# cornell-zhang/HiSparse

Measured on AMD Instinct MI355X. Metric: SpMV GBPS (8 B per non-zero per SpMV, sw/benchmark.cpp:312-346), higher is better.
Workload: dtype u32 (Q8.24 fixed point, u64 row sums)

## Files before the change

hisparse_amd/csrc/spmv_bitmap.hip:

```cpp
#include <hip/hip_runtime.h>

#include <cstdio>
#include <cstdlib>
#include <vector>

#include "spmv_device.h"
#include "spmv_kernels.h"

namespace hisparse {
namespace dev {

namespace {

constexpr int kBmThreads = kWaveLanes * kBitmapWaves;
constexpr int kBatch = 8;
constexpr uint32_t kInvalidOffset = 0x80000000u;
constexpr uint32_t kRsrcFlags = 0x00020000u;
constexpr int kXCopyPasses = (kBitmapMaxXLdsGroups * (kBitmapGroupCols / 4) + kBmThreads - 1) / kBmThreads;

typedef const __attribute__((address_space(4))) WaveSeg* WaveSegTable;

template <bool kFloat>
struct Batch {
    uint32_t v[kBatch], xv[kBatch];
    uint64_t m[kBatch];
};

typedef const __attribute__((address_space(3))) uint32_t* LdsWords;

template <typename T>
__device__ __forceinline__ T* uniform_ptr(T* p) {
    const uint64_t v = reinterpret_cast<uint64_t>(p);
    const uint32_t hi = static_cast<uint32_t>(__builtin_amdgcn_readfirstlane(static_cast<uint32_t>(v >> 32)));
    const uint32_t lo = static_cast<uint32_t>(__builtin_amdgcn_readfirstlane(static_cast<uint32_t>(v)));
    return reinterpret_cast<T*>((static_cast<uint64_t>(hi) << 32) | lo);
}

template <bool kFloat, int kAblate, bool kXLds>
__device__ __forceinline__ typename Rows<kFloat>::sum_t bitmap_row_run(const uint64_t* mp, const uint32_t*& vp, const uint32_t* x, uint32_t num_cols,
                                                                       uint32_t col0, uint32_t steps, uint32_t lane, bool have_first,
                                                                       const uint32_t (&first_masks)[4], LdsWords xs_run, uint64_t* stamps = nullptr) {
    using R = Rows<kFloat>;
    typename R::sum_t acc = 0;
    const auto vr = __builtin_amdgcn_make_buffer_rsrc(uniform_ptr(const_cast<uint32_t*>(vp)), 0, 0x7fffffffu, kRsrcFlags);
    uint32_t xk[kBatch];
#pragma unroll
    for (int k = 0; k < kBatch; ++k) xk[k] = (lane + k * kBitmapGroupCols) * 4u;
    uint32_t voff = 0;
    const auto mr = __builtin_amdgcn_make_buffer_rsrc(uniform_ptr(const_cast<uint64_t*>(mp)), 0, steps * 8u, kRsrcFlags);
    uint32_t moff = lane < 2 * kBatch ? lane * 4u : kInvalidOffset;
    constexpr uint32_t kBatchMaskBytes = kBatch * 8u;
    uint32_t mcur = have_first ? first_masks[0] : __builtin_amdgcn_raw_buffer_load_b32(mr, moff, 0, 0);
    uint32_t m1 = have_first ? first_masks[1] : __builtin_amdgcn_raw_buffer_load_b32(mr, moff + kBatchMaskBytes, 0, 0);
    uint32_t m2 = have_first ? first_masks[2] : __builtin_amdgcn_raw_buffer_load_b32(mr, moff + 2 * kBatchMaskBytes, 0, 0);
    uint32_t m3 = have_first ? first_masks[3] : __builtin_amdgcn_raw_buffer_load_b32(mr, moff + 3 * kBatchMaskBytes, 0, 0);
    auto issue = [&](Batch<kFloat>& b, uint32_t bb) {
        constexpr uint32_t sel = 0;
        const uint32_t xc = min(col0 + bb * (kBatch * kBitmapGroupCols), num_cols);
        const auto xr = __builtin_amdgcn_make_buffer_rsrc(const_cast<uint32_t*>(x + xc), 0, (num_cols - xc) * 4u, kRsrcFlags);
#pragma unroll
        for (int k = 0; k < kBatch; ++k) {
            const uint32_t lo = __builtin_amdgcn_readlane(mcur, sel + 2 * k), hi = __builtin_amdgcn_readlane(mcur, sel + 2 * k + 1);
            b.m[k] = (static_cast<uint64_t>(hi) << 32) | lo;
            const uint32_t off = __builtin_amdgcn_mbcnt_hi(hi, __builtin_amdgcn_mbcnt_lo(lo, 0)) * 4u;
            b.v[k] = (kAblate & 1) ? off : __builtin_amdgcn_raw_buffer_load_b32(vr, off, voff, (kAblate & 256) ? 2 : 0);
            if constexpr (kXLds) b.xv[k] = (kAblate & 2) ? lo : xs_run[(bb * kBatch + k) * kBitmapGroupCols + lane];
            else b.xv[k] = (kAblate & 2) ? lo : __builtin_amdgcn_raw_buffer_load_b32(xr, xk[k], 0, 0);
            const uint32_t set = static_cast<uint32_t>(__builtin_popcountll(b.m[k]));
            asm("s_lshl2_add_u32 %0, %1, %2" : "=s"(voff) : "s"(set), "s"(__builtin_amdgcn_readfirstlane(voff)) : "scc");
// ... 49 lines not shown
        rotate_masks(bb + 2);
        issue(A, bb + 2);
        consume(B);
        rotate_masks(bb + 3);
        issue(B, bb + 3);
    }
    vp += voff / 4u;
    return acc;
}

template <bool kFloat, int kAblate, bool kXLds = false>
__global__ __launch_bounds__(kBmThreads) void spmv_bitmap_kernel(const uint8_t* __restrict__ image, const Block* __restrict__ blocks,
                                                                const Unit* __restrict__ units, const uint32_t* __restrict__ x, uint32_t num_cols,
                                                                uint32_t* __restrict__ out, int32_t row_part_filter,
                                                                const uint32_t* __restrict__ part_heads, uint64_t* __restrict__ timeline,
                                                                uint32_t x_lds_offset, CarriedCombine carry) {
    using R = Rows<kFloat>;
    using acc_t = typename R::acc_t;
    extern __shared__ __attribute__((aligned(16))) uint8_t lds[];
    acc_t* ys = reinterpret_cast<acc_t*>(lds);
    const uint32_t tid = threadIdx.x;
    const uint32_t lane = tid & (kWaveLanes - 1);
    const uint32_t wave = __builtin_amdgcn_readfirstlane(tid / kWaveLanes);
    uint64_t* stamps = (kAblate & 64) ? timeline + (static_cast<size_t>(blockIdx.x) * kBitmapWaves + wave) * 8 : nullptr;
    auto stamp = [&](int i, uint32_t dep) {
        if (!(kAblate & 64)) return;
        uint64_t t;
        asm volatile("s_memrealtime %0\n\ts_waitcnt lgkmcnt(0)" : "=s"(t) : "s"(dep));
        if (lane == 0) stamps[i] = t;
    };
    stamp(0, wave);
    uint32_t wg = blockIdx.x;
    if ((gridDim.x & 7u) == 0) wg = (blockIdx.x & 7u) * (gridDim.x >> 3) + (blockIdx.x >> 3);
    if (carry.partial) carried_combine<kFloat, kBmThreads>(carry, blockIdx.x, gridDim.x, tid);
    uint32_t bi = wg;
    if (row_part_filter >= 0) {
        bi = ((const __attribute__((address_space(4))) uint32_t*)part_heads)[static_cast<uint32_t>(row_part_filter) * gridDim.x + wg];
        if (bi == kNoBlock) return;
    }
    bool first_block = true;
    uint32_t staged_col0 = 0, staged_groups = 0;
    for (uint32_t next = 0;; bi = next) {
        const BlockTable blk = (BlockTable)(blocks + bi);
        next = (row_part_filter >= 0 && blk->next_part > static_cast<uint32_t>(row_part_filter)) ? 0u : blk->next;
        const uint32_t nrows = blk->nrows, out0 = blk->out_offset;
        const uint32_t* hdr = reinterpret_cast<const uint32_t*>(units) + (static_cast<size_t>(bi) * kBitmapWaves + wave) * (kBitmapRunSlots * 16);
        const uint32_t seg_word = hdr[min(lane, 15u)];
        uint32_t first_masks[4];
#pragma unroll
        for (int b = 0; b < 4; ++b) first_masks[b] = hdr[16 + 16 * b + (lane & 15u)];
        const uint32_t row_begin = __builtin_amdgcn_readlane(seg_word, 0), row_end = __builtin_amdgcn_readlane(seg_word, 1);
        const uint32_t g_begin = __builtin_amdgcn_readlane(seg_word, 2), steps = __builtin_amdgcn_readlane(seg_word, 3) - g_begin;
        const uint64_t* mp = reinterpret_cast<const uint64_t*>(image) +
                             ((static_cast<uint64_t>(__builtin_amdgcn_readlane(seg_word, 7)) << 32) | __builtin_amdgcn_readlane(seg_word, 6));
        const uint32_t* vp = reinterpret_cast<const uint32_t*>(image) +
                             ((static_cast<uint64_t>(__builtin_amdgcn_readlane(seg_word, 5)) << 32) | __builtin_amdgcn_readlane(seg_word, 4));
        const uint32_t col0 = blk->first_col0 + g_begin * kBitmapGroupCols;
        stamp(1, col0 + steps + nrows);

        if (!first_block) __syncthreads();
        for (uint32_t i = tid; i <= nrows; i += kBmThreads) ys[i] = 0;
        LdsWords xs_run = nullptr;
        if constexpr (kXLds) {
            const uint32_t c0 = blk->first_col0, groups = blk->first_ncols;
            typedef uint32_t u4 __attribute__((ext_vector_type(4)));
            auto* xs = (__attribute__((address_space(3))) u4*)(lds + x_lds_offset);
            if (first_block || c0 != staged_col0 || groups != staged_groups) {
// ... 107 lines not shown
```

hisparse_amd/csrc/spmv_device.h:

```cpp
#ifndef HISPARSE_SPMV_DEVICE_H_
#define HISPARSE_SPMV_DEVICE_H_

#include <hip/hip_runtime.h>

#include <type_traits>

#include "stream_tiles.h"

namespace hisparse {
namespace dev {
namespace {

__device__ __forceinline__ uint32_t q8_24_mul(uint32_t a, uint32_t b) {
    const uint64_t wide = static_cast<uint64_t>(a) * b + 0x800000ull;
    uint32_t hi = static_cast<uint32_t>(wide >> 32);
    const uint32_t lo = static_cast<uint32_t>(wide);
    asm("" : "+v"(hi));
    const uint32_t r = __builtin_amdgcn_alignbit(hi, lo, 24);
    return (hi >> 24) ? 0xffffffffu : r;
}

typedef const __attribute__((address_space(4))) Unit* UnitTable;
typedef const __attribute__((address_space(4))) Block* BlockTable;

// ... 70 lines not shown
template <typename T>
__device__ __forceinline__ T segmented_run_sums(T v, uint32_t row, bool& is_last) {
    segmented_step<0x111, 0xf>(v, row);
    segmented_step<0x112, 0xf>(v, row);
    segmented_step<0x114, 0xf>(v, row);
    segmented_step<0x118, 0xf>(v, row);
    segmented_step<0x142, 0xa>(v, row);
    segmented_step<0x143, 0xc>(v, row);
    const uint32_t next_row = static_cast<uint32_t>(__builtin_amdgcn_update_dpp(-1, static_cast<int>(row), 0x130, 0xf, 0xf, false));
    is_last = next_row != row;
    return v;
}


struct CarriedCombine {
    const uint32_t* partial = nullptr;
    uint32_t* y = nullptr;
    uint32_t num_rows = 0;
    uint32_t slices = 0;
};

template <typename Launch>
inline CarriedCombine carried(const Launch& a) {
    CarriedCombine c;
    if (a.carry_partial && a.carry_slices > 1 && a.row_part_filter < 0) {
        c.partial = a.carry_partial;
        c.y = a.carry_y;
        c.num_rows = a.carry_rows;
        c.slices = a.carry_slices;
    }
    return c;
}

template <bool kFloat, int kBlockThreads>
__device__ __forceinline__ void carried_combine(const CarriedCombine& c, uint32_t wg, uint32_t groups, uint32_t tid) {
    using Sum = typename std::conditional<kFloat, float, uint32_t>::type;
    const uint32_t quads = c.num_rows / 4u, per = (quads + groups - 1u) / groups;
    const uint32_t q_end = min(quads, (wg + 1u) * per);
    for (uint32_t q = wg * per + tid; q < q_end; q += kBlockThreads) {
        const uint4* p = reinterpret_cast<const uint4*>(c.partial) + q;
        Sum s[4] = {0, 0, 0, 0};
        for (uint32_t k0 = 0; k0 < c.slices; k0 += 4u) {
            uint4 v[4];
#pragma unroll
            for (uint32_t k = 0; k < 4u; ++k) v[k] = p[static_cast<size_t>(min(k0 + k, c.slices - 1u)) * quads];
#pragma unroll
            for (uint32_t k = 0; k < 4u; ++k) {
                if (k0 + k >= c.slices) break;
                const uint32_t w[4] = {v[k].x, v[k].y, v[k].z, v[k].w};
#pragma unroll
                for (int j = 0; j < 4; ++j) {
                    if constexpr (kFloat) s[j] += __uint_as_float(w[j]);
                    else s[j] = __builtin_elementwise_add_sat(s[j], w[j]);
                }
            }
        }
        uint4 out;
        if constexpr (kFloat) out = make_uint4(__float_as_uint(s[0]), __float_as_uint(s[1]), __float_as_uint(s[2]), __float_as_uint(s[3]));
        else out = make_uint4(s[0], s[1], s[2], s[3]);
        reinterpret_cast<uint4*>(c.y)[q] = out;
    }
}

}
}
}

#endif
```

hisparse_amd/csrc/spmv_kernels.hip:

```cpp
#include <hip/hip_runtime.h>

#include <cstdio>
#include <cstdlib>
#include <utility>
#include <vector>

#include "spmv_kernels.h"
#include "spmv_device.h"

namespace hisparse {
namespace dev {

namespace {

constexpr int kThreads = kWaveLanes * kWavesPerWorkgroup;
constexpr int kLightThreads = 256;
#ifndef HS_LIGHT_BATCH
#define HS_LIGHT_BATCH 4
#endif
constexpr int kLightBatch = HS_LIGHT_BATCH;
constexpr uint32_t kBufBytes = kSubTileCols * 4u;

template <int kIters, int kStride>
__device__ __forceinline__ void fill_x(uint32_t* dst, const uint32_t* __restrict__ x, uint32_t col0, uint32_t ncols, uint32_t t) {
    const uint4* src = reinterpret_cast<const uint4*>(x + col0);
    uint4* d = reinterpret_cast<uint4*>(dst);
    const uint32_t n4 = ncols / 4;
    uint4 r[kIters];
#pragma unroll
    for (int j = 0; j < kIters; ++j) r[j] = src[min(t + j * kStride, n4 - 1)];
#pragma unroll
    for (int j = 0; j < kIters; ++j) d[min(t + j * kStride, n4 - 1)] = r[j];
}

constexpr uint32_t kDmaCols = kWaveLanes * 4;
constexpr uint32_t kDmaPerFill = kSubTileCols / kDmaCols / kLoaderWaves;
__device__ __forceinline__ void dma_fill_x(uint32_t* dst, const uint32_t* __restrict__ x, uint32_t col0, uint32_t ncols, uint32_t w,
                                           uint32_t lane) {
#pragma unroll
    for (uint32_t j = 0; j < kDmaPerFill; ++j) {
        const uint32_t c = (w * kDmaPerFill + j) * kDmaCols;
        __builtin_amdgcn_global_load_lds((const __attribute__((address_space(1))) uint32_t*)(x + col0 + min(c + lane * 4, ncols - 4)),
                                         (__attribute__((address_space(3))) uint32_t*)(dst + c), 16, 0, 0);
    }
}
template <int kFills>
__device__ __forceinline__ void dma_wait() {
    asm volatile("s_waitcnt vmcnt(%0)" ::"n"(kFills * kDmaPerFill) : "memory");
}

#ifndef HS_ROWBLOCK_STREAM_POLICY
#define HS_ROWBLOCK_STREAM_POLICY "nt"
#endif
#ifndef HS_ROWBLOCK_RESIDENT_POLICY
#define HS_ROWBLOCK_RESIDENT_POLICY "sc1"
#endif
#define HS_BY_POLICY(kRes, STATEMENT)                                 \
    do {                                                              \
        if constexpr (kRes) { STATEMENT(HS_ROWBLOCK_RESIDENT_POLICY); } \
        else { STATEMENT(HS_ROWBLOCK_STREAM_POLICY); }                \
    } while (0)
#define HS_RING_AGPRS "a0", "a1", "a2", "a3", "a4", "a5", "a6", "a7", "a8", "a9", "a10", "a11", "a12", "a13", "a14", "a15", "a16", "a17", \
                      "a18", "a19", "a20", "a21", "a22", "a23", "a24", "a25", "a26", "a27", "a28", "a29", "a30", "a31"
constexpr int kMaxDepth = 16;
constexpr int kOwner24Depth = 3;

constexpr int ring_format(int kRing) { return (kRing & 8) ? 4 : (kRing & 3); }
constexpr bool ring_is_delta(int kRing) { return ring_format(kRing) == 1 || ring_format(kRing) == 4; }
template <int kFmt, bool kRes>
struct RingT;
template <int kRing>
using Ring = RingT<ring_format(kRing), (kRing & 4) != 0>;
template <bool kRes>
struct RingT<0, kRes> {
    static constexpr uint32_t kLaneBytes = 8;
    template <int K>
    static __device__ __forceinline__ void issue(const uint8_t* base, uint32_t byte_off, uint32_t lane_off) {
#define HS_ISSUE(P) asm volatile("s_nop 4\n\tglobal_load_dwordx2 a[%0:%1], %2, %3 " P ::"n"(2 * K), "n"(2 * K + 1), "v"(byte_off + lane_off), "s"(base) : "memory", HS_RING_AGPRS)
        HS_BY_POLICY(kRes, HS_ISSUE);
#undef HS_ISSUE
    }
    template <int K, int kDepth>
    static __device__ __forceinline__ void take(uint32_t& value, uint32_t& where) {
        asm volatile("s_waitcnt vmcnt(%4)\n\tv_accvgpr_read_b32 %0, a[%2]\n\tv_accvgpr_read_b32 %1, a[%3]"
                     : "=v"(value), "=v"(where) : "n"(2 * K), "n"(2 * K + 1), "n"(kDepth - 1) : "memory");
    }
    template <int K, int kDepth>
    static __device__ __forceinline__ void take2(uint32_t& value0, uint32_t& where0, uint32_t& value1, uint32_t& where1) {
        asm volatile("s_waitcnt vmcnt(%8)\n\tv_accvgpr_read_b32 %0, a[%4]\n\tv_accvgpr_read_b32 %1, a[%5]\n\tv_accvgpr_read_b32 %2, a[%6]\n\t"
                     "v_accvgpr_read_b32 %3, a[%7]"
                     : "=v"(value0), "=v"(where0), "=v"(value1), "=v"(where1)
                     : "n"(2 * K), "n"(2 * K + 1), "n"(2 * K + 2), "n"(2 * K + 3), "n"(kDepth - 2) : "memory");
    }
};
template <bool kRes>
struct RingT<1, kRes> {
    static constexpr uint32_t kLaneBytes = 8;
    template <int K>
    static __device__ __forceinline__ void issue(const uint8_t* base, uint32_t byte_off, uint32_t lane_off) {
        static_assert(2 * K + 1 < kMaxDepth && K + kMaxDepth < 2 * kMaxDepth, "values in a0..a15, gap words in a16..a23: ring depth <= 8");
// ... 536 lines not shown
template <bool kFloat, int kRing, int kAblate, int kDepth, bool kOwner = false>
__device__ __forceinline__ void rowblock_workgroup(const uint8_t* __restrict__ image, const Block* __restrict__ blocks,
                                                   const Unit* __restrict__ units, const uint32_t* __restrict__ x,
                                                   uint32_t* __restrict__ out, int32_t row_part_filter, uint32_t ring,
                                                   uint32_t x_base, const uint32_t* __restrict__ part_heads, const CarriedCombine& carry) {
    using acc_t = typename Rows<kFloat>::acc_t;
    extern __shared__ __attribute__((aligned(16))) uint8_t lds[];
    acc_t* ys = reinterpret_cast<acc_t*>(lds);
    uint32_t* xs = reinterpret_cast<uint32_t*>(lds + x_base);
    const uint32_t tid = threadIdx.x;
    const uint32_t lane = tid & (kWaveLanes - 1);
    const uint32_t wave = __builtin_amdgcn_readfirstlane(tid / kWaveLanes);
    const bool loader = wave >= kConsumerWaves;
    uint32_t wg = blockIdx.x;
    if ((gridDim.x & 7u) == 0) wg = (blockIdx.x & 7u) * (gridDim.x >> 3) + (blockIdx.x >> 3);

    uint32_t bi = wg;
    if (row_part_filter >= 0) {
        bi = ((const __attribute__((address_space(4))) uint32_t*)part_heads)[static_cast<uint32_t>(row_part_filter) * gridDim.x + wg];
        if (bi == kNoBlock) return;
    }
    bool first_block = true;
    uint32_t block_no = 0;
    for (uint32_t next = 0;; bi = next, ++block_no) {
        const BlockTable blk = (BlockTable)(blocks + bi);
        next = (row_part_filter >= 0 && blk->next_part > static_cast<uint32_t>(row_part_filter)) ? 0u : blk->next;
        const uint32_t nrows = blk->nrows, out0 = blk->out_offset;
        const UnitTable unit = (UnitTable)(units + blk->unit_begin);
        const uint32_t U = blk->unit_end - blk->unit_begin;

        if (!first_block) __syncthreads();
        first_block = false;
        timeline_stamp<kAblate>(block_no, wave, lane, 0);
        Consumer<kFloat> c;
        if (!loader && U > 0) {
            if constexpr (kRing == 3)
                consumer_begin_owner24<kFloat, kDepth>(c, image + blk->wave_offset[wave], unit, U, wave, lane, xs, ring, ys, nrows, blk->total_steps[wave], blk->first_end[wave]);
            else
                consumer_begin<kFloat, kRing, kDepth, kOwner>(c, image + blk->wave_offset[wave], unit, U, wave, lane, xs, ring, ys, nrows, blk->total_steps[wave],
                                                               blk->first_end[wave]);
            if constexpr (ring_format(kRing) == 4) c.value_shift = blk->value_shift;
        }
        if (carry.partial && block_no == 0) carried_combine<kFloat, kThreads>(carry, blockIdx.x, gridDim.x, tid);
        if (kOwner) {
            if (!(kAblate & 16)) for (uint32_t i = tid; i < nrows + kConsumerWaves; i += kThreads) reinterpret_cast<float*>(ys)[i] = 0.0f;
        } else
        if (!(kAblate & 16)) for (uint32_t i = tid; i <= nrows; i += kThreads) ys[i] = 0;
        if (U > 0 && !(kAblate & 16)) fill_x<kSubTileCols / 4 / kThreads, kThreads>(xs, x, blk->first_col0, blk->first_ncols, tid);
        __syncthreads();
        timeline_stamp<kAblate>(block_no, wave, lane, 1);

        if (U > 0) {
            if (loader) {
                const uint32_t lw = wave - kConsumerWaves;
                __builtin_amdgcn_s_setprio(3);
                uint32_t fill_slot = 1 == ring ? 0 : 1;
                uint32_t col0_next = U > 1 ? unit[1].col0 : 0, ncols_next = U > 1 ? unit[1].ncols : 8;
                uint32_t col0_after = U > 2 ? unit[2].col0 : col0_next, ncols_after = U > 2 ? unit[2].ncols : ncols_next;
                auto refill = [&](uint32_t v) {
                    const uint32_t col0 = col0_next, ncols = ncols_next;
                    if (kOwner) {
                        col0_next = col0_after;
                        ncols_next = ncols_after;
                        const uint32_t ahead = min(v + 2, U - 1);
                        col0_after = unit[ahead].col0;
                        ncols_after = unit[ahead].ncols;
                    } else {
                        const uint32_t ahead = min(v + 1, U - 1);
                        col0_next = unit[ahead].col0;
                        ncols_next = unit[ahead].ncols;
                    }
                    if (!(kAblate & 4)) dma_fill_x(xs + fill_slot * kSubTileCols, x, col0, ncols, lw, lane);
                    fill_slot = fill_slot + 1 == ring ? 0 : fill_slot + 1;
                };
                uint32_t issued = 1;
                while (issued < U && issued < ring - 1) refill(issued++);
                uint64_t t_wait = 0, t_bar = 0, t_issue = 0;
                const uint64_t t_begin = (kOwner && (kAblate & 256)) ? __builtin_readcyclecounter() : 0;
                for (uint32_t u = 0; u < U; ++u) {
                    const uint64_t ti = (kOwner && (kAblate & 256)) ? __builtin_readcyclecounter() : 0;
                    if (issued < U) refill(issued++);
// ... 533 lines not shown
```

hisparse_amd/csrc/spmv_sweep.hip:

```cpp
#include <hip/hip_runtime.h>

#include <utility>

#include "spmv_device.h"
#include "spmv_kernels.h"

namespace hisparse {
namespace dev {

namespace {

constexpr int kSweepThreads = kSweepWaves * kWaveLanes;
#ifndef HS_SWEEP_DEPTH
#define HS_SWEEP_DEPTH 4
#endif
constexpr int kSweepDepth = HS_SWEEP_DEPTH;

__device__ __forceinline__ const uint8_t* sweep_scalar_pointer(const void* p) {
    const uint64_t a = reinterpret_cast<uint64_t>(p);
    const uint32_t hi = __builtin_amdgcn_readfirstlane(static_cast<uint32_t>(a >> 32));
    const uint32_t lo = __builtin_amdgcn_readfirstlane(static_cast<uint32_t>(a));
    return reinterpret_cast<const uint8_t*>((static_cast<uint64_t>(hi) << 32) | lo);
}

// ... 117 lines not shown
#pragma unroll
            for (uint32_t k = 0; k < kRowsInFlight; ++k)
                if (base + k * kSweepThreads < nrows) out[base + k * kSweepThreads] = __float_as_uint(static_cast<float>(v[k]));
        } else {
            uint32_t sum[kRowsInFlight], flags[kRowsInFlight];
            const uint32_t flag0 = SweepRows<false>::flag_word0(nrows);
#pragma unroll
            for (uint32_t k = 0; k < kRowsInFlight; ++k) {
                const uint32_t row = min(base + k * kSweepThreads, nrows);
                sum[k] = acc[row];
                flags[k] = acc[flag0 + (row >> 5)];
            }
            asm volatile("" ::: "memory");
#pragma unroll
            for (uint32_t k = 0; k < kRowsInFlight; ++k) {
                const uint32_t row = base + k * kSweepThreads;
                if (row < nrows) out[row] = ((flags[k] >> (row & 31u)) & 1u) ? 0xffffffffu : sum[k];
            }
        }
    }
}

template <bool kFloat, int kAblate, bool kNt>
__global__ __launch_bounds__(kSweepThreads) void spmv_sweep_kernel(const uint8_t* __restrict__ image, const Block* __restrict__ blocks,
                                                                  const uint32_t* __restrict__ x, uint32_t* __restrict__ out,
                                                                  int32_t row_part_filter, const uint32_t* __restrict__ part_heads, CarriedCombine carry) {
    using R = SweepRows<kFloat>;
    extern __shared__ __attribute__((aligned(16))) uint8_t lds[];
    uint8_t* ys = lds;
    const uint32_t tid = threadIdx.x, lane = tid & (kWaveLanes - 1);
    const uint32_t wave = __builtin_amdgcn_readfirstlane(tid / kWaveLanes);
    uint32_t wg = blockIdx.x;
    if ((gridDim.x & 7u) == 0) wg = (blockIdx.x & 7u) * (gridDim.x >> 3) + (blockIdx.x >> 3);
    if (carry.partial) carried_combine<kFloat, kSweepThreads>(carry, blockIdx.x, gridDim.x, tid);
    uint32_t bi = wg;
    if (row_part_filter >= 0) {
        bi = ((const __attribute__((address_space(4))) uint32_t*)part_heads)[static_cast<uint32_t>(row_part_filter) * gridDim.x + wg];
        if (bi == kNoBlock) return;
    }
    const uint8_t* xs = sweep_scalar_pointer(x);
    const uint32_t lane_off = lane * 8u;
    bool first_block = true;
    for (uint32_t next = 0;; bi = next) {
        const BlockTable blk = (BlockTable)(blocks + bi);
        next = (row_part_filter >= 0 && blk->next_part > static_cast<uint32_t>(row_part_filter)) ? 0u : blk->next;
        const uint32_t nrows = blk->nrows, out0 = blk->out_offset, steps = blk->total_steps[0], pad_col = blk->first_col0;
        const uint8_t* stream = sweep_scalar_pointer(image + blk->wave_offset[0] + uint64_t(wave) * kChunkBytes);
        const __attribute__((address_space(4))) uint32_t* bases =
            (const __attribute__((address_space(4))) uint32_t*)(image + blk->wave_offset[1]) + uint64_t(wave) * steps;
        SweepLane st;
#pragma unroll
        for (int k = 0; k < kSweepDepth; ++k) { st.value[k] = 0; st.row[k] = nrows; }
        if (steps) sweep_prime<(kAblate & 8) != 0, kNt>(std::make_integer_sequence<int, kSweepDepth>(), stream, xs, pad_col, steps, lane_off);
        if (!first_block) __syncthreads();
        first_block = false;
        if (!(kAblate & 4)) sweep_zero_rows(ys, R::lds_words(nrows), tid);
        __syncthreads();
        if (steps) {
            const uint32_t last = steps - 1;
            uint32_t b[kSweepDepth];
#pragma unroll
            for (int k = 0; k < kSweepDepth; ++k) b[k] = bases[min(uint32_t(k), last)];
            for (uint32_t s0 = 0; s0 < steps + kSweepDepth; s0 += kSweepDepth) {
                uint32_t nb[kSweepDepth];
#pragma unroll
                for (int k = 0; k < kSweepDepth; ++k) nb[k] = bases[min(s0 + kSweepDepth + k, last)];
                sweep_round<kFloat, kAblate, kNt>(std::make_integer_sequence<int, kSweepDepth>(), st, stream, xs, s0, steps, steps + kSweepDepth, lane_off, b, ys, nrows);
// ... 60 lines not shown
```

hisparse_amd/csrc/stream_plan.h:

```cpp
#ifndef HISPARSE_STREAM_PLAN_H_
#define HISPARSE_STREAM_PLAN_H_

#include <algorithm>
#include <cmath>
#include <cstdint>
#include <cstdio>
#include <cstdlib>
#include <functional>
#include <map>
#include <numeric>
#include <string>
#include <vector>

#include "stream_tiles.h"
#include "tiles_common.h"

namespace hisparse {
namespace dev {
namespace detail {

enum class ForcedFormat { kNone, kPairs, kDelta, kOwner, kOwner24, kSweep, kBitmap, kInvalid };
struct IntSwitch {
    bool set = false;
    int value = 0;
// ... 276 lines not shown
    p.best = 1e30;
    for (uint32_t cs = 1; cs <= (force_slices ? kMaxForcedColSlices : kMaxColSlices); ++cs) {
        const uint32_t live_tiles = (num_cols + kSubTileCols - 1) / kSubTileCols;
        if (force_slices ? uint32_t(in.sw.col_slices.value) != cs : (!owner && (cs & (cs - 1)) != 0 && live_tiles > 2 * kMaxColSlices && in.sw.pow2_slices)) continue;
        if (cs > 1 && uint64_t(CP) * S < cs) continue;
        if (!force_slices && !owner && live_tiles <= kMaxColSlices && cs > live_tiles) continue;
        for (const Shape& shape : (cs > 1 || owner) ? std::vector<Shape>(sliced, sliced + 2) : std::vector<Shape>(whole, whole + 1)) {
            uint32_t cap = shape.cap, ring = shape.ring;
            if (force_rows) {
                cap = std::min<uint32_t>(cap, std::max(1, in.sw.max_rows.value));
                ring = std::max(kMinXBuffers, std::min(kMaxXBuffers, (kMaxLdsBytes - (cap + spare_rows) * acc_bytes) / (kSubTileCols * 4u)));
            }
            const uint64_t per_round = std::max<uint32_t>(1, G / cs);
            const uint64_t need = (uint64_t(num_rows) + cap - 1) / cap;
            const double ranges = double(per_round * std::max<uint64_t>(1, (need + per_round - 1) / per_round));
            const double blocks_per_wg = ranges * cs / G;
            const uint64_t memo_key = (uint64_t(ranges) << 8) | cs;
            auto found = census_memo.find(memo_key);
            if (found == census_memo.end()) found = census_memo.emplace(memo_key, census.evaluate(uint64_t(ranges), cs, G, nnz)).first;
            const TileCensus::Eval& real = found->second;
            const double units_per_wg = std::max(1.0, real.nonempty_units / G);
            const double unit_stream_us = double(nnz) * 8.0 / (units_per_wg * G) / 25e3;
            const double volume_us = real.nonempty_units * double(L.sub_width) * 4.0 / G / (owner ? 29e3 : 120e3);
            double latency_us = units_per_wg * std::max(0.0, 0.8 / (ring - 1) - unit_stream_us);
            if (!owner && cs == 1) latency_us += units_per_wg * 0.3;
            if (!owner && cs > 1 && live_tiles <= 2 * kMaxColSlices)
                latency_us += 0.75 * (double(nnz) * 8.0 / G / 25e3) * (double((live_tiles + cs - 1) / cs) * cs / live_tiles - 1.0);
            const double rows_per_block = double(num_rows) / ranges, per_row_and_tile = double(nnz) / std::max(1.0, double(num_rows) * sub_tiles * census.populated);
            if (!owner && rows_per_block <= kDenseBlockRows && per_row_and_tile < 4.0 * kWaveLanes) latency_us += units_per_wg * 1.75;
            const double lanes_per_row = std::min(64.0, 896.0 / std::max(1.0, rows_per_block));
            const bool pairs_likely = !delta || (!format_forced && double(nnz) * 1.6 < double(is_float ? kDeltaMinSavedBytesFloat : kDeltaMinSavedBytes));
            const double conflict_us = (!owner && pairs_likely && lanes_per_row > 1.0 && per_row_and_tile >= 16.0)
                                           ? double(nnz) / G / kWaveLanes * (lanes_per_row - 1.0) * 2.0 / 2400.0 : 0.0;
            const bool carried = double(nnz) * 8.1 < double(kCarryMaxImageBytes);
            const double combine_us = cs > 1 ? (carried ? 1.0 : 3.5) + double(num_rows) * 4.0 * (cs + 1) / 4e6 : 0.0;
            const double uniform_load = double(nnz) / std::max(1.0, ranges * cs) * std::ceil(blocks_per_wg);
            const double idle_us = double(nnz) * 8.0 / 6.2e6 * ((std::ceil(blocks_per_wg) / std::max(1e-9, blocks_per_wg) - 1.0) +
                                                                 std::max(0.0, real.max_wg_load / std::max(1.0, uniform_load) - 1.15) * uniform_load / std::max(1.0, double(nnz) / G));
            const double cost = volume_us + latency_us + conflict_us + 8.0 * blocks_per_wg + combine_us + idle_us;
            if (in.sw.debug)
                std::fprintf(stderr, "plan cs %u cap %u ring %u: ranges %.0f volume %.1f latency %.1f conflicts %.1f blocks/wg %.2f idle %.2f combine %.1f => %.2f us\n", cs, cap, ring, ranges,
                             volume_us, latency_us, conflict_us, blocks_per_wg, idle_us, combine_us, cost);
            if (cost < p.best) { p.best = cost; p.best_units = real.nonempty_units; p.slices = cs; p.max_rows = cap; }
        }
    }
}

inline TilePlan plan_row_blocks(const PlanInputs& in, double hub_share, DenseRowChoice dense, bool owner_allowed) {
    const uint32_t num_rows = in.L.num_rows, num_cols = in.L.num_cols, max_workgroups = in.max_workgroups;
    const uint64_t nnz = in.nnz;
    TilePlan p;
    bool keep_delta_for_hubs = false;
    p.format = choose_stream_format(in, hub_share, dense.prefer_sliced_delta, owner_allowed, keep_delta_for_hubs);
    p.light = choose_light(in, dense, p.format);
    for (int attempt = 0; attempt < 2; ++attempt) {
        p.format_forced = in.sw.format_set() || dense.prefer_sliced_delta || (keep_delta_for_hubs && p.format == kFormatDelta);
        uint32_t light_wgs = kLightWorkgroupsPerCu;
        if (in.sw.light_wgs.set) light_wgs = std::min<uint32_t>(6u, std::max(1, in.sw.light_wgs.value));
        p.G = std::max<uint32_t>(1, max_workgroups) * (p.light ? light_wgs : 1u);
        p.slices = 1;
        p.max_rows = p.light ? kLightMaxBlockRows : max_block_rows(false);
        if (p.light) {
            if (in.sw.max_rows.set) p.max_rows = std::min<uint32_t>(p.max_rows, std::max(1, in.sw.max_rows.value));
        } else {
            cost_row_block_plans(in, p);
        }
        if (attempt == 0 && !p.owner() && !p.light && !p.format_forced && !in.sw.sweep.set && !in.sw.col_slices.set && !in.sw.max_rows.set &&
// ... 74 lines not shown
```

hisparse_amd/csrc/stream_tiles.h:

```cpp
#ifndef HISPARSE_STREAM_TILES_H_
#define HISPARSE_STREAM_TILES_H_

#include <cstdint>
#include <string>
#include <memory>
#include <utility>
#include <vector>

#include "hisparse/common.h"

namespace hisparse {
namespace dev {

constexpr uint32_t kWaveLanes = 64;
constexpr uint32_t kWavesPerWorkgroup = 16;
constexpr uint32_t kConsumerWaves = 14;
constexpr uint32_t kLoaderWaves = kWavesPerWorkgroup - kConsumerWaves;
constexpr uint32_t kSubTileCols = 8192;
constexpr uint32_t kMaxXBuffers = 4;
constexpr uint32_t kMinXBuffers = 2;
constexpr uint32_t kAccumulatorBytes = 8;
constexpr uint32_t max_block_rows(bool sliced) { return (sliced ? 96u : 32u) * 1024u / kAccumulatorBytes - 1u; }
constexpr uint32_t kMaxColSlices = 8;
constexpr uint32_t kMaxForcedColSlices = 16;
constexpr uint32_t kMaxSweepSlices = 16;
constexpr uint64_t kCarryMaxImageBytes = 160ull << 20;
constexpr uint64_t kSlicedDeltaMaxImageBytes = 48ull << 20;
constexpr uint64_t kResidentMaxImageBytes = 256ull << 20;
constexpr uint64_t kRowblockResidentMaxImageBytes = 256ull << 20;
constexpr uint64_t kRowblockResidentSmallImageBytes = 32ull << 20;
constexpr uint32_t kMaxLdsBytes = 160 * 1024;
constexpr uint32_t kChunkBytes = kWaveLanes * 8;
constexpr uint32_t kWaveStrideBytes = kChunkBytes * kConsumerWaves;
constexpr uint32_t kRecordBytes = kWaveLanes * 2 * (4 + 2);
constexpr uint32_t kRecordBytes24 = kWaveLanes * (3 + 3 + 2 + 2);
constexpr uint32_t kMaxValueShift = 8;
constexpr uint64_t kDelta24OutlierShare = 4096;
constexpr uint64_t kDelta24MinSavedBytes = 23u << 20;
constexpr uint32_t delta_record_bytes(uint32_t value_bits) { return value_bits == 24 ? kRecordBytes24 : kRecordBytes; }
constexpr bool value_fits24(uint32_t word, uint32_t shift) { return (word >> shift) < (1u << 24) && (word & ((1u << shift) - 1u)) == 0; }
struct Outlier { uint32_t row, col, value; };
enum class DeltaValueBits : uint32_t { kByRule = 0, kPacked = 24, kPlain = 32 };
constexpr uint32_t kMaxGap = 0xfffeu;
constexpr uint32_t kBridgeGap = 0xffffu;
constexpr uint32_t kBridgeAdvance = 0xffffu;
constexpr double kDeltaMinMeanGap = 8.0;
constexpr double kDeltaMaxMeanGap = 20000.0;
constexpr uint64_t kDeltaMinSavedBytes = 23u << 20;
constexpr uint64_t kDeltaMinSavedBytesFloat = 40u << 20;
constexpr double kDenseMeanGap = 320.0;
enum StreamFormat : uint32_t { kFormatPairs = 0, kFormatDelta = 1, kFormatBitmap = 2, kFormatOwner = 3, kFormatPairs24 = 4, kFormatOwner24 = 5, kFormatSweep = 6 };
constexpr bool rowblock_stream(uint32_t format, bool light) { return (format == kFormatPairs || format == kFormatDelta) && !light; }
constexpr bool stream_policy_applies(uint32_t format, bool light) { return format == kFormatSweep || rowblock_stream(format, light); }
constexpr bool plan_stream_resident(uint32_t format, bool light, uint64_t image_bytes, uint64_t num_units, uint64_t num_blocks) {
    return rowblock_stream(format, light)
               ? image_bytes <= kRowblockResidentMaxImageBytes && (num_units > num_blocks || image_bytes <= kRowblockResidentSmallImageBytes)
               : image_bytes <= kResidentMaxImageBytes;
}
constexpr bool plan_carries(uint32_t format, uint64_t image_bytes) {
// ... 159 lines not shown
```

hisparse_amd/csrc/sweep_tiles.cpp:

```cpp
#include <algorithm>
#include <atomic>
#include <cmath>
#include <cstdio>
#include <cstring>
#include <memory>
#include <mutex>
#include <numeric>

#include "gpu_tiles.h"
#include "hisparse/q8_24.h"
#include "tiles_common.h"

namespace hisparse {
namespace dev {

using namespace detail;

namespace {

constexpr double kSweepNsPerElementResident = 0.27, kSweepNsPerElementStreamed = 0.38, kSweepNsPerLine = 0.66, kSweepBlockUs = 4.2;
constexpr double kSweepCutNsPerElement = 0.33, kSweepCutNsPerLine = 1.36;

struct Placed { uint64_t key; uint32_t value; };

}

double sweep_plan(const Layout& L, uint64_t nnz, uint32_t max_workgroups, uint32_t& slices, uint64_t& want_ranges, uint32_t& max_rows) {
    const uint32_t num_rows = L.num_rows, num_cols = L.num_cols;
    const uint32_t G = std::max<uint32_t>(1, max_workgroups);
    max_rows = L.g->impl == IMPL_FIXED ? kSweepMaxBlockRowsFixed : kSweepMaxBlockRowsFloat;
    if (const char* v = env_switch("HISPARSE_SPMM_VECTORS")) if (std::atoi(v) == 4) max_rows = std::max(1u, max_rows / 4u - 1u);
    if (const char* force = env_switch("HISPARSE_MAX_ROWS")) max_rows = std::min<uint32_t>(max_rows, std::max(1, std::atoi(force)));
    const uint64_t by_cap = detail::ranges_by_cap(L, max_rows);
    const uint32_t lines = (num_cols + kSweepColAlign - 1) / kSweepColAlign;
    const char* force_slices = env_switch("HISPARSE_COL_SLICES");
    double best = 1e30;
    slices = 1;
    want_ranges = 1;
    for (uint32_t cs = 1; cs <= std::min<uint32_t>(kMaxSweepSlices, std::max<uint32_t>(1, lines)); ++cs) {
        if (force_slices && uint32_t(std::atoi(force_slices)) != cs) continue;
        if (uint64_t(cs) * num_rows > 0xffffffffull) continue;
        const uint64_t per_round = std::max<uint32_t>(1, G / cs);
        const uint64_t rounds = std::max<uint64_t>(1, (by_cap + per_round - 1) / per_round);
        const uint64_t ranges = std::min<uint64_t>(per_round * rounds, std::max<uint64_t>(by_cap, std::max<uint64_t>(1, nnz / 4096)));
        const double blocks = double(ranges) * cs, blocks_per_wg = std::ceil(blocks / G);
        if (cs > kMaxColSlices && !force_slices && double(nnz) / blocks < 32768.0) continue;
        const double per_element = double(nnz) * 8.1 <= double(kResidentMaxImageBytes) ? kSweepNsPerElementResident : kSweepNsPerElementStreamed;
        const double block_ns = double(nnz) / blocks * per_element + double(lines) / cs * kSweepNsPerLine;
        const double combine_us = double(num_rows) * 4.0 * cs / 4e6 + (cs > 1 ? 2.0 + double(num_rows) * 4.0 * (cs + 1) / 8e6 : 0.0);
        const double cost = blocks_per_wg * (block_ns * 1e-3 + kSweepBlockUs) + combine_us;
        if (env_switch("HISPARSE_PLAN_DEBUG")) std::fprintf(stderr, "sweep plan cs %u: ranges %llu block %.1f us combine %.1f => %.1f us\n", cs, (unsigned long long)ranges, block_ns * 1e-3, combine_us, cost);
        if (cost < best) { best = cost; slices = cs; want_ranges = ranges; }
    }
    return best;
}

bool build_sweep_tiles(const Layout& L, const void* const channel[NUM_HBM_CHANNELS], const uint64_t n_packets[NUM_HBM_CHANNELS],
                       const std::vector<uint32_t>& row_nnz, uint32_t max_workgroups, StreamTiles& out, std::string& error, const CsrView* csr_in,
                       GpuTiler* gpu, uint64_t image_slack) {
    const uint32_t num_rows = L.num_rows, num_cols = L.num_cols, RP = L.row_parts, CP = L.col_parts;
    const uint32_t G = std::max<uint32_t>(1, max_workgroups);
    auto chan = [&](uint32_t pc) { return static_cast<const MatPkt*>(channel[pc]); };
    if (uint64_t(num_cols) * 4 >= (1ull << 32)) { error = "sweep: x does not fit a 32-bit byte offset"; return false; }
    PhaseTimer timer;

    std::vector<uint64_t> row_ptr(size_t(num_rows) + 1, 0);
    for (uint32_t r = 0; r < num_rows; ++r) row_ptr[r + 1] = row_ptr[r] + row_nnz[r];
    const uint64_t nnz = row_ptr[num_rows];
    std::unique_ptr<uint64_t[]> elems_buf;
    uint64_t* elems = nullptr;
    auto rows_on_the_host = [&]() -> bool {
    if (elems) return true;
    elems_buf.reset(new uint64_t[std::max<uint64_t>(nnz, 1)]);
    elems = elems_buf.get();
    if (csr_in) {
        const HostCsr csr(csr_in);
        if (!csr.ok()) { error = "CSR column index outside the matrix"; return false; }
        const bool fixed = L.g->impl == IMPL_FIXED;
        std::atomic<bool> bad_column(false);
// ... 247 lines not shown
```

Before: 7255.

## Issue carried-combine slice loads early and overlap with x-tile fill

```diff
diff --git a/hisparse_amd/csrc/spmv_bitmap.hip b/hisparse_amd/csrc/spmv_bitmap.hip
--- a/hisparse_amd/csrc/spmv_bitmap.hip
+++ b/hisparse_amd/csrc/spmv_bitmap.hip
@@ -27,14 +27,6 @@
 };
 
 typedef const __attribute__((address_space(3))) uint32_t* LdsWords;
-
-template <typename T>
-__device__ __forceinline__ T* uniform_ptr(T* p) {
-    const uint64_t v = reinterpret_cast<uint64_t>(p);
-    const uint32_t hi = static_cast<uint32_t>(__builtin_amdgcn_readfirstlane(static_cast<uint32_t>(v >> 32)));
-    const uint32_t lo = static_cast<uint32_t>(__builtin_amdgcn_readfirstlane(static_cast<uint32_t>(v)));
-    return reinterpret_cast<T*>((static_cast<uint64_t>(hi) << 32) | lo);
-}
 
 template <bool kFloat, int kAblate, bool kXLds>
 __device__ __forceinline__ typename Rows<kFloat>::sum_t bitmap_row_run(const uint64_t* mp, const uint32_t*& vp, const uint32_t* x, uint32_t num_cols,
@@ -150,7 +142,11 @@
     stamp(0, wave);
     uint32_t wg = blockIdx.x;
     if ((gridDim.x & 7u) == 0) wg = (blockIdx.x & 7u) * (gridDim.x >> 3) + (blockIdx.x >> 3);
-    if (carry.partial) carried_combine<kFloat, kBmThreads>(carry, blockIdx.x, gridDim.x, tid);
+    if (carry.partial) {
+        CarryLoads<kCarryBatch> carried_rows;
+        carried_issue<kBmThreads>(carry, blockIdx.x, gridDim.x, tid, carried_rows);
+        carried_finish<kFloat, kBmThreads>(carry, carried_rows);
+    }
     uint32_t bi = wg;
     if (row_part_filter >= 0) {
         bi = ((const __attribute__((address_space(4))) uint32_t*)part_heads)[static_cast<uint32_t>(row_part_filter) * gridDim.x + wg];
diff --git a/hisparse_amd/csrc/spmv_device.h b/hisparse_amd/csrc/spmv_device.h
--- a/hisparse_amd/csrc/spmv_device.h
+++ b/hisparse_amd/csrc/spmv_device.h
@@ -126,33 +126,78 @@
     return c;
 }
 
-template <bool kFloat, int kBlockThreads>
-__device__ __forceinline__ void carried_combine(const CarriedCombine& c, uint32_t wg, uint32_t groups, uint32_t tid) {
+constexpr uint32_t kCarryBatch = kMaxColSlices;
+typedef uint32_t CarryPair __attribute__((ext_vector_type(2)));
+template <uint32_t kBatch>
+struct CarryLoads {
+    CarryPair v[kBatch];
+    uint32_t p, p_end;
+};
+constexpr uint32_t kCarryRsrcFlags = 0x00020000u;
+constexpr uint32_t kCarryNoLoad = 0xfffffff8u;
+
+template <typename T>
+__device__ __forceinline__ T* uniform_ptr(T* p) {
+    const uint64_t v = reinterpret_cast<uint64_t>(p);
+    const uint32_t hi = static_cast<uint32_t>(__builtin_amdgcn_readfirstlane(static_cast<uint32_t>(v >> 32)));
+    const uint32_t lo = static_cast<uint32_t>(__builtin_amdgcn_readfirstlane(static_cast<uint32_t>(v)));
+    return reinterpret_cast<T*>((static_cast<uint64_t>(hi) << 32) | lo);
+}
+
+template <uint32_t kBatch>
+__device__ __forceinline__ void carry_load_batch(const CarriedCombine& c, CarryLoads<kBatch>& l, uint32_t k0) {
+    uint32_t rows = c.num_rows;
+    asm volatile("" : "+s"(rows));
+    const uint32_t off = l.p < l.p_end ? l.p * 8u : kCarryNoLoad;
+#pragma unroll
+    for (uint32_t k = 0; k < kBatch; ++k) {
+        const uint32_t slice_no = min(k0 + k, c.slices - 1u);
+        const auto slice = __builtin_amdgcn_make_buffer_rsrc(uniform_ptr(const_cast<uint32_t*>(c.partial + static_cast<size_t>(slice_no) * rows)), 0, rows * 4u, kCarryRsrcFlags);
+        l.v[k] = __builtin_amdgcn_raw_buffer_load_b64(slice, k0 + k < c.slices ? off : kCarryNoLoad, 0, 0);
+    }
+}
+
+template <bool kFloat, uint32_t kBatch>
+__device__ __forceinline__ void carry_finish_round(const CarriedCombine& c, CarryLoads<kBatch>& l) {
     using Sum = typename std::conditional<kFloat, float, uint32_t>::type;
-    const uint32_t quads = c.num_rows / 4u, per = (quads + groups - 1u) / groups;
-    const uint32_t q_end = min(quads, (wg + 1u) * per);
-    for (uint32_t q = wg * per + tid; q < q_end; q += kBlockThreads) {
-        const uint4* p = reinterpret_cast<const uint4*>(c.partial) + q;
-        Sum s[4] = {0, 0, 0, 0};
-        for (uint32_t k0 = 0; k0 < c.slices; k0 += 4u) {
-            uint4 v[4];
+    Sum s0 = 0, s1 = 0;
+    for (uint32_t k0 = 0;;) {
 #pragma unroll
-            for (uint32_t k = 0; k < 4u; ++k) v[k] = p[static_cast<size_t>(min(k0 + k, c.slices - 1u)) * quads];
-#pragma unroll
-            for (uint32_t k = 0; k < 4u; ++k) {
-                if (k0 + k >= c.slices) break;
-                const uint32_t w[4] = {v[k].x, v[k].y, v[k].z, v[k].w};
-#pragma unroll
-                for (int j = 0; j < 4; ++j) {
-                    if constexpr (kFloat) s[j] += __uint_as_float(w[j]);
-                    else s[j] = __builtin_elementwise_add_sat(s[j], w[j]);
-                }
+        for (uint32_t k = 0; k < kBatch; ++k) {
+            if constexpr (kFloat) {
+                s0 += __uint_as_float(l.v[k].x);
+                s1 += __uint_as_float(l.v[k].y);
+            } else {
+                s0 = __builtin_elementwise_add_sat(s0, l.v[k].x);
+                s1 = __builtin_elementwise_add_sat(s1, l.v[k].y);
             }
         }
-        uint4 out;
-        if constexpr (kFloat) out = make_uint4(__float_as_uint(s[0]), __float_as_uint(s[1]), __float_as_uint(s[2]), __float_as_uint(s[3]));
-        else out = make_uint4(s[0], s[1], s[2], s[3]);
-        reinterpret_cast<uint4*>(c.y)[q] = out;
+        k0 += kBatch;
+        if (k0 >= c.slices) break;
+        carry_load_batch(c, l, k0);
+    }
+    CarryPair out;
+    if constexpr (kFloat) { out.x = __float_as_uint(s0); out.y = __float_as_uint(s1); }
+    else { out.x = s0; out.y = s1; }
+    if (l.p < l.p_end) reinterpret_cast<CarryPair*>(c.y)[l.p] = out;
+}
+
+template <int kBlockThreads, uint32_t kBatch>
+__device__ __forceinline__ void carried_issue(const CarriedCombine& c, uint32_t wg, uint32_t groups, uint32_t tid, CarryLoads<kBatch>& l) {
+    const uint32_t quads = c.num_rows / 4u, per = (quads + groups - 1u) / groups;
+    asm volatile("" : "+v"(tid));
+    l.p = 2u * min(quads, wg * per) + tid;
+    l.p_end = 2u * min(quads, (wg + 1u) * per);
+    carry_load_batch(c, l, 0);
+    asm volatile("" ::: "memory");
+}
+
+template <bool kFloat, int kBlockThreads, uint32_t kBatch>
+__device__ __forceinline__ void carried_finish(const CarriedCombine& c, CarryLoads<kBatch>& l) {
+    carry_finish_round<kFloat>(c, l);
+    for (l.p += kBlockThreads; l.p < l.p_end; l.p += kBlockThreads) {
+        carry_load_batch(c, l, 0);
+        carry_finish_round<kFloat>(c, l);
     }
 }
 
diff --git a/hisparse_amd/csrc/spmv_kernels.hip b/hisparse_amd/csrc/spmv_kernels.hip
--- a/hisparse_amd/csrc/spmv_kernels.hip
+++ b/hisparse_amd/csrc/spmv_kernels.hip
@@ -21,14 +21,18 @@
 constexpr int kLightBatch = HS_LIGHT_BATCH;
 constexpr uint32_t kBufBytes = kSubTileCols * 4u;
 
+typedef uint32_t XQuad __attribute__((ext_vector_type(4)));
 template <int kIters, int kStride>
-__device__ __forceinline__ void fill_x(uint32_t* dst, const uint32_t* __restrict__ x, uint32_t col0, uint32_t ncols, uint32_t t) {
-    const uint4* src = reinterpret_cast<const uint4*>(x + col0);
-    uint4* d = reinterpret_cast<uint4*>(dst);
+__device__ __forceinline__ void fill_x_load(XQuad (&r)[kIters], const uint32_t* __restrict__ x, uint32_t col0, uint32_t ncols, uint32_t t) {
+    const XQuad* src = reinterpret_cast<const XQuad*>(x + col0);
     const uint32_t n4 = ncols / 4;
-    uint4 r[kIters];
 #pragma unroll
     for (int j = 0; j < kIters; ++j) r[j] = src[min(t + j * kStride, n4 - 1)];
+}
+template <int kIters, int kStride>
+__device__ __forceinline__ void fill_x_store(uint32_t* dst, const XQuad (&r)[kIters], uint32_t ncols, uint32_t t) {
+    XQuad* d = reinterpret_cast<XQuad*>(dst);
+    const uint32_t n4 = ncols / 4;
 #pragma unroll
     for (int j = 0; j < kIters; ++j) d[min(t + j * kStride, n4 - 1)] = r[j];
 }
@@ -54,6 +58,9 @@
 #endif
 #ifndef HS_ROWBLOCK_RESIDENT_POLICY
 #define HS_ROWBLOCK_RESIDENT_POLICY "sc1"
+#endif
+#ifndef HS_CARRY_LOADS_FIRST
+#define HS_CARRY_LOADS_FIRST 1
 #endif
 #define HS_BY_POLICY(kRes, STATEMENT)                                 \
     do {                                                              \
@@ -66,6 +73,7 @@
 constexpr int kOwner24Depth = 3;
 
 constexpr int ring_format(int kRing) { return (kRing & 8) ? 4 : (kRing & 3); }
+constexpr uint32_t carry_batch(bool is_float, int kRing) { return (kRing & 3) == 3 || is_float ? 4u : 5u; }
 constexpr bool ring_is_delta(int kRing) { return ring_format(kRing) == 1 || ring_format(kRing) == 4; }
 template <int kFmt, bool kRes>
 struct RingT;
@@ -668,6 +676,16 @@
         if (!first_block) __syncthreads();
         first_block = false;
         timeline_stamp<kAblate>(block_no, wave, lane, 0);
+        constexpr int kFillIters = kSubTileCols / 4 / kThreads;
+        const bool carry_here = carry.partial && block_no == 0, fill_here = U > 0 && !(kAblate & 16);
+        constexpr bool kCarryApart = (kRing & 3) == 3;
+        CarryLoads<carry_batch(kFloat, kRing)> carried_rows;
+        XQuad x_tile[kFillIters];
+        if (HS_CARRY_LOADS_FIRST) {
+            if (carry_here) carried_issue<kThreads>(carry, blockIdx.x, gridDim.x, tid, carried_rows);
+            if (carry_here && kCarryApart) carried_finish<kFloat, kThreads>(carry, carried_rows);
+            if (fill_here) fill_x_load<kFillIters, kThreads>(x_tile, x, blk->first_col0, blk->first_ncols, tid);
+        }
         Consumer<kFloat> c;
         if (!loader && U > 0) {
             if constexpr (kRing == 3)
@@ -677,12 +695,17 @@
                                                                blk->first_end[wave]);
             if constexpr (ring_format(kRing) == 4) c.value_shift = blk->value_shift;
         }
-        if (carry.partial && block_no == 0) carried_combine<kFloat, kThreads>(carry, blockIdx.x, gridDim.x, tid);
+        if (!HS_CARRY_LOADS_FIRST) {
+            if (carry_here) carried_issue<kThreads>(carry, blockIdx.x, gridDim.x, tid, carried_rows);
+            if (carry_here && kCarryApart) carried_finish<kFloat, kThreads>(carry, carried_rows);
+            if (fill_here) fill_x_load<kFillIters, kThreads>(x_tile, x, blk->first_col0, blk->first_ncols, tid);
+        }
         if (kOwner) {
             if (!(kAblate & 16)) for (uint32_t i = tid; i < nrows + kConsumerWaves; i += kThreads) reinterpret_cast<float*>(ys)[i] = 0.0f;
         } else
         if (!(kAblate & 16)) for (uint32_t i = tid; i <= nrows; i += kThreads) ys[i] = 0;
-        if (U > 0 && !(kAblate & 16)) fill_x<kSubTileCols / 4 / kThreads, kThreads>(xs, x, blk->first_col0, blk->first_ncols, tid);
+        if (fill_here) fill_x_store<kFillIters, kThreads>(xs, x_tile, blk->first_ncols, tid);
+        if (carry_here && !kCarryApart) carried_finish<kFloat, kThreads>(carry, carried_rows);
         __syncthreads();
         timeline_stamp<kAblate>(block_no, wave, lane, 1);
 
diff --git a/hisparse_amd/csrc/spmv_sweep.hip b/hisparse_amd/csrc/spmv_sweep.hip
--- a/hisparse_amd/csrc/spmv_sweep.hip
+++ b/hisparse_amd/csrc/spmv_sweep.hip
@@ -173,7 +173,11 @@
     const uint32_t wave = __builtin_amdgcn_readfirstlane(tid / kWaveLanes);
     uint32_t wg = blockIdx.x;
     if ((gridDim.x & 7u) == 0) wg = (blockIdx.x & 7u) * (gridDim.x >> 3) + (blockIdx.x >> 3);
-    if (carry.partial) carried_combine<kFloat, kSweepThreads>(carry, blockIdx.x, gridDim.x, tid);
+    if (carry.partial) {
+        CarryLoads<kCarryBatch> carried_rows;
+        carried_issue<kSweepThreads>(carry, blockIdx.x, gridDim.x, tid, carried_rows);
+        carried_finish<kFloat, kSweepThreads>(carry, carried_rows);
+    }
     uint32_t bi = wg;
     if (row_part_filter >= 0) {
         bi = ((const __attribute__((address_space(4))) uint32_t*)part_heads)[static_cast<uint32_t>(row_part_filter) * gridDim.x + wg];
diff --git a/hisparse_amd/csrc/stream_plan.h b/hisparse_amd/csrc/stream_plan.h
--- a/hisparse_amd/csrc/stream_plan.h
+++ b/hisparse_amd/csrc/stream_plan.h
@@ -332,7 +332,7 @@
             const bool pairs_likely = !delta || (!format_forced && double(nnz) * 1.6 < double(is_float ? kDeltaMinSavedBytesFloat : kDeltaMinSavedBytes));
             const double conflict_us = (!owner && pairs_likely && lanes_per_row > 1.0 && per_row_and_tile >= 16.0)
                                            ? double(nnz) / G / kWaveLanes * (lanes_per_row - 1.0) * 2.0 / 2400.0 : 0.0;
-            const bool carried = double(nnz) * 8.1 < double(kCarryMaxImageBytes);
+            const bool carried = double(nnz) * 8.1 < double(kCarryPricedMaxImageBytes);
             const double combine_us = cs > 1 ? (carried ? 1.0 : 3.5) + double(num_rows) * 4.0 * (cs + 1) / 4e6 : 0.0;
             const double uniform_load = double(nnz) / std::max(1.0, ranges * cs) * std::ceil(blocks_per_wg);
             const double idle_us = double(nnz) * 8.0 / 6.2e6 * ((std::ceil(blocks_per_wg) / std::max(1e-9, blocks_per_wg) - 1.0) +
diff --git a/hisparse_amd/csrc/stream_tiles.h b/hisparse_amd/csrc/stream_tiles.h
--- a/hisparse_amd/csrc/stream_tiles.h
+++ b/hisparse_amd/csrc/stream_tiles.h
@@ -25,6 +25,7 @@
 constexpr uint32_t kMaxForcedColSlices = 16;
 constexpr uint32_t kMaxSweepSlices = 16;
 constexpr uint64_t kCarryMaxImageBytes = 160ull << 20;
+constexpr uint64_t kCarryPricedMaxImageBytes = 160ull << 20;
 constexpr uint64_t kSlicedDeltaMaxImageBytes = 48ull << 20;
 constexpr uint64_t kResidentMaxImageBytes = 256ull << 20;
 constexpr uint64_t kRowblockResidentMaxImageBytes = 256ull << 20;
diff --git a/hisparse_amd/csrc/sweep_tiles.cpp b/hisparse_amd/csrc/sweep_tiles.cpp
--- a/hisparse_amd/csrc/sweep_tiles.cpp
+++ b/hisparse_amd/csrc/sweep_tiles.cpp
@@ -44,7 +44,8 @@
         const uint64_t rounds = std::max<uint64_t>(1, (by_cap + per_round - 1) / per_round);
         const uint64_t ranges = std::min<uint64_t>(per_round * rounds, std::max<uint64_t>(by_cap, std::max<uint64_t>(1, nnz / 4096)));
         const double blocks = double(ranges) * cs, blocks_per_wg = std::ceil(blocks / G);
-        if (cs > kMaxColSlices && !force_slices && double(nnz) / blocks < 32768.0) continue;
+        const bool carried = double(nnz) * 8.1 < double(kCarryPricedMaxImageBytes);
+        if (cs > kMaxColSlices && !force_slices && double(nnz) / blocks < 32768.0 && !carried) continue;
         const double per_element = double(nnz) * 8.1 <= double(kResidentMaxImageBytes) ? kSweepNsPerElementResident : kSweepNsPerElementStreamed;
         const double block_ns = double(nnz) / blocks * per_element + double(lines) / cs * kSweepNsPerLine;
         const double combine_us = double(num_rows) * 4.0 * cs / 4e6 + (cs > 1 ? 2.0 + double(num_rows) * 4.0 * (cs + 1) / 8e6 : 0.0);
```

Result: no change. 7313 (median of 5 runs) (+0.8%).
